# lauraset/Super-resolution-building-height-estimation

Measured on AMD Instinct MI355X. Metric: tiles/sec (64x64x8ch->256x256 height), higher is better.
Workload: dtype f16 operands / f32 accumulate (MFMA), f32 residual stream; 1 GPU; RRDBNet x4 (23 RRDB, 64 feat) forward_feature, batch 32 tiles/GPU, 64x64x3 -> 64x256x256 (BASELINE.json configs[1]); global_batch=32, parallelism=tile-sharded x1 (no data-path collective)

## Files before the change

### include/srbh.h

```cpp
#ifndef SRBH_H
#define SRBH_H

#include <stddef.h>
#include <stdint.h>

#ifdef __cplusplus
extern "C" {
#endif

#define SRBH_OK 0
#define SRBH_ERR_ARG (-1)
#define SRBH_ERR_WORKSPACE (-2)

int srbh_version(void);
const char* srbh_last_error(void);
#define SRBH_PATH_HCONV16 0
#define SRBH_PATH_HCONV_TEMPLATE 1
#define SRBH_PATH_ENTRY_FUSED 2
#define SRBH_PATH_ENTRY_SPLIT 3
#define SRBH_PATH_WGRAD16 4
#define SRBH_PATH_WGRAD_B16_GENERIC 5
#define SRBH_PATH_WGRAD_F32 6
#define SRBH_PATH_WGRAD_ENTRY_FUSED 7
#define SRBH_PATH_WGRAD_ENTRY_SPLIT 8
// ... 108 lines not shown
int srbh_rrdbnet_trunk_train_forward_persistent(const srbh_rrdbnet_desc* d, float* xr, float* xrr, void* dense_all, size_t dense_stride, int B, int H,
                                                int W, void* aux, void* stream, int* used);
size_t srbh_rrdbnet_trunk_wgrad_ws_bytes(void);
int srbh_rrdbnet_trunk_train_backward(int num_block, const void* dense_all, size_t dense_stride, const void* packs, size_t pack_stride,
                                      const size_t* pack_off, float* g_a, float* g_b, float* g_c, float** g_out, void* G, size_t g_stride,
                                      float* dw_all, float* db_all, float* wgrad_ws, int B, int H, int W, void* stream);
int srbh_rrdbnet_trunk_train_backward_persistent(int num_block, const void* dense_all, size_t dense_stride, const void* packs, size_t pack_stride,
                                                 const size_t* pack_off, const float* zero_bias, const float* g_a, float* g_b, float* g_c,
                                                 float** g_out, void* G_all, size_t g_stride, float* dw_all, float* db_all, float* wgrad_ws,
                                                 void* trunk_wgrad_ws, int B, int H, int W, void* aux, void* stream, int* used);
size_t srbh_trunk_wgrad_ws_bytes(int num_block, int B, int H, int W);
int srbh_trunk_wgrad(int num_block, const void* dense_all, size_t dense_stride, const void* G_all, size_t g_stride, int B, int H, int W, float* dw_all,
                     float* db_all, void* ws, void* stream);

int srbh_rrdbnet_last_status(const void* ws, int B, int H, int W, int want_forward, void* stream);

int srbh_rrdbnet_trunk_out(const void* ws, size_t ws_bytes, int num_block, int B, int H, int W, int want_forward, float* out, void* stream);

int srbh_ptail_wgs_cap(int cap);

int srbh_trunk_timing(int on);
int srbh_trunk_last_ms(float* ms);
const char* srbh_trunk_kernel_name(void);

size_t srbh_hpack_bytes(int cout, int cin, int ksize);
int srbh_hpack_conv_f32(const float* w_oihw, int cout, int cin, int ksize, int transpose_flip, float* packed, void* stream);

size_t srbh_bn_stats_bytes(int C);
int srbh_hconv_up_supported(int H, int W);

// ... 295 lines not shown
```

### super-resolution-building-height-estimation_amd/_lib.py

```python
from __future__ import annotations

import ctypes as C
import os
import subprocess
import threading

_HERE = os.path.dirname(os.path.abspath(__file__))
ROOT = os.path.dirname(_HERE)
CSRC = os.path.join(_HERE, "csrc")
INCLUDE = os.path.join(ROOT, "include")
LIB_PATH = os.path.join(_HERE, "libsrbh.so")
_DEV_LIB = os.environ.get("SRBH_LIB_PATH")
SOURCES = ["srbh_conv3x3.hip", "srbh_aux.hip", "srbh_rrdbnet.hip", "srbh_ptrunk.hip", "srbh_trunk_wgrad.hip", "srbh_ptail.hip", "srbh_ptail_split.hip", "srbh_head.hip", "srbh_head_bwd.hip", "srbh_mosaic.hip", "srbh_loader.hip", "srbh_loss.hip", "srbh_dwconv.hip", "srbh_mbconv.hip", "srbh_pwconv.hip", "srbh_dconv.hip", "srbh_optim.hip"]
HIPCC = os.environ.get("HIPCC", "/opt/rocm/bin/hipcc")
HIPFLAGS = ["--offload-arch=gfx950", "-O3", "-std=c++17", "-fPIC", "-Wno-unused-result", "-Wno-inline-asm"]
if os.environ.get("SRBH_HIPFLAGS_OVERRIDE"):
    HIPFLAGS = os.environ["SRBH_HIPFLAGS_OVERRIDE"].split()


def build(force: bool = False, verbose: bool = False) -> str:
    srcs = [os.path.join(CSRC, s) for s in SOURCES if os.path.exists(os.path.join(CSRC, s))]
    deps = srcs + [os.path.join(CSRC, f) for f in os.listdir(CSRC) if f.endswith(".h")] + [os.path.join(INCLUDE, "srbh.h")]
    if not force and os.path.exists(LIB_PATH) and all(os.path.getmtime(LIB_PATH) >= os.path.getmtime(d) for d in deps):
        return LIB_PATH
# ... 251 lines not shown
    "srbh_transpose_many": (_i, [_vp, _i, _vp]),
    "srbh_pwconv_bwd_data": (_i, [_vp, _vp, _vp, _i, _i, _i, _i, _vp]),
    "srbh_pwconv_bwd_data_res": (_i, [_vp, _vp, _vp, _vp, _i, _i, _i, _i, _vp]),
    "srbh_pwconv_bwd_weight_ws_floats": (_sz, [_i, _i, _i, _i]),
    "srbh_pwconv_bwd_weight": (_i, [_vp, _vp, _vp, _vp, _i, _i, _i, _i, _vp]),
    "srbh_dwconv_fwd": (_i, [_vp, _vp, _vp] + [_i] * 10 + [_vp]),
    "srbh_dwconv_bwd_data": (_i, [_vp, _vp, _vp] + [_i] * 10 + [_vp]),
    "srbh_dwconv_bwd_weight_splits": (_i, [_i, _i]),
    "srbh_dwconv_bwd_weight": (_i, [_vp, _vp, _vp, _vp] + [_i] * 10 + [_vp]),
    "srbh_mosaic_accumulate": (_i, [_vp, _vp, _i, _i, _i, _i, _vp, _vp, _vp, _vp, _i, _i, _vp]),
    "srbh_mosaic_finalize": (_i, [_vp, _vp, _vp, _i, _i, _i, _vp, _vp, _vp]),
    "srbh_label_prep": (_i, [_vp, _i, _i, _i, _vp, _vp, _vp, _vp, _vp, _vp, _vp, _vp]),
    "srbh_normalize_clamp": (_i, [_vp, _vp, _i, _i, _i, _i, _vp, _vp, _f, _f, _i, _vp]),
    "srbh_rrdbnet_workspace_bytes": (_sz, [_i, _i, _i, _i]),
    "srbh_rrdbnet_last_status": (_i, [_vp, _i, _i, _i, _i, _vp]),
    "srbh_rrdbnet_trunk_out": (_i, [_vp, _sz, _i, _i, _i, _i, _i, _vp, _vp]),
    "srbh_ptail_wgs_cap": (_i, [_i]),
    "srbh_wmse_sum": (_i, [_vp, _vp, _vp, C.c_long, _vp, _vp]),
    "srbh_wmse_grad": (_i, [_vp, _vp, _vp, C.c_long, _vp, _vp, _vp]),
    "srbh_cedice_sums": (_i, [_vp, _i, _i, C.c_long, C.c_long, C.c_long, C.c_long, _vp, _vp, _vp, _vp]),
    "srbh_cedice_grad": (_i, [_vp, _i, _i, C.c_long, C.c_long, C.c_long, C.c_long, _vp, _vp, _vp, _vp, _vp]),
    "srbh_height_metric_sums": (_i, [_vp, _vp, _vp, C.c_long, _i, _vp, _vp]),
    "srbh_confusion_add": (_i, [_vp, _vp, C.c_long, _i, _vp, _vp, _vp]),
    "srbh_trunk_timing": (_i, [_i]),
    "srbh_trunk_last_ms": (_i, [C.POINTER(C.c_float)]),
    "srbh_trunk_kernel_name": (C.c_char_p, []),
    "srbh_rrdbnet_forward": (_i, [C.POINTER(RRDBNetDesc), _vp, _vp, _i, _i, _i, _i, _vp, _sz, _vp]),
}

_lib = None
# ... 50 lines not shown
```

### super-resolution-building-height-estimation_amd/csrc/srbh_aux.hip

```cpp
#include "srbh_internal.h"

namespace srbh {

static thread_local char g_err[512] = "";

unsigned long long g_path_counters[PATH_N] = {};
void set_error(const char* fmt, ...) {
    va_list ap;
    va_start(ap, fmt);
    vsnprintf(g_err, sizeof(g_err), fmt, ap);
    va_end(ap);
}

int hip_fail(hipError_t e, const char* what) {
    set_error("HIP error %d (%s) in %s", (int)e, hipGetErrorString(e), what);
    return (int)e;
}

__global__ void zero_words_kernel(unsigned* __restrict__ p, size_t n) {
    size_t i = (size_t)blockIdx.x * blockDim.x + threadIdx.x;
    const size_t stride = (size_t)gridDim.x * blockDim.x;
    for (; i < n; i += stride) p[i] = 0u;
}

// ... 156 lines not shown
#pragma unroll
    for (int k = 0; k < 8; ++k) {
        float a = acc[k];
#pragma unroll
        for (int m = 4; m < 64; m <<= 1) a += __shfl_xor(a, m);
        if ((threadIdx.x & 63) < 4) atomicAdd(&red[oct * 8 + k], a);
    }
    __syncthreads();
    if (threadIdx.x < 32) atomicAdd(out + chunk * 32 + threadIdx.x, red[threadIdx.x]);
}

template <int CIN, int BF16 = 0>
__global__ __launch_bounds__(256) void conv_first_kernel(const float* __restrict__ x, const float* __restrict__ w,
                                                         const float* __restrict__ bias, int B, int cin_rt, int H, int W,
                                                         float* ra, float* rb, float* rc, char* out16, int row_b,
                                                         int plane_b, long img_b) {
    extern __shared__ float s_w[];
    const int cin = CIN > 0 ? CIN : cin_rt;
    for (int u = threadIdx.x; u < cin * 9 * 64; u += 256) {
        const int oc = u & 63, k = u >> 6;
        s_w[u] = w[(long)oc * cin * 9 + k];
    }
    __syncthreads();
    const int wq = (W + 3) >> 2;
    const long idx = (long)blockIdx.x * 256 + threadIdx.x;
    const long total = (long)B * H * wq * 16;
    if (idx >= total) return;
    const int og = idx & 15;
    long r = idx >> 4;
    const int xg = r % wq; r /= wq;
    const int yy = r % H;
    const int b = r / H;
// ... 278 lines not shown
    const int gx = (int)((npix + 255) / 256 < 1024 ? (npix + 255) / 256 : 1024);
    const char* base = (const char*)src + (long)chunk0 * g.plane_b;
    if (bf16) hipLaunchKernelGGL(act16_channel_sum_kernel<1>, dim3(gx, nchunk), dim3(256), 0, (hipStream_t)stream, base, B, H, W, nchunk, g.row_b, g.plane_b, g.img_b, out);
    else hipLaunchKernelGGL(act16_channel_sum_kernel<0>, dim3(gx, nchunk), dim3(256), 0, (hipStream_t)stream, base, B, H, W, nchunk, g.row_b, g.plane_b, g.img_b, out);
    SRBH_HIP(hipGetLastError());
    return SRBH_OK;
}

extern "C" int srbh_conv_first_f32(const float* x, const float* w, const float* bias, int B, int cin, int H, int W,
                                   float* ra, float* rb, float* rc, void* out16, int out16_chunks_total,
                                   void* stream) {
    return srbh::conv_first_f32(x, w, bias, B, cin, H, W, ra, rb, rc, out16, out16_chunks_total, 0, stream);
}

int srbh::conv_first_f32(const float* x, const float* w, const float* bias, int B, int cin, int H, int W, float* ra, float* rb, float* rc,
                         void* out16, int out16_chunks_total, int bf16, void* stream) {
    SRBH_REQUIRE(x && w && B > 0 && cin > 0 && H > 0 && W > 0, "srbh_conv_first_f32: bad arguments");
    SRBH_REQUIRE(!out16 || out16_chunks_total >= 2, "srbh_conv_first_f32: out16 needs >= 2 chunk planes");
    Act16Geo g = act16_geo(B, out16_chunks_total > 0 ? out16_chunks_total : 2, H, W);
    SRBH_REQUIRE(cin <= 56, "srbh_conv_first_f32: at most 56 input channels (got %d)", cin);
    long total = (long)B * H * ((W + 3) / 4) * 16;
    const size_t lds = (size_t)cin * 9 * 64 * sizeof(float);
    if (cin == 3 && bf16)
        hipLaunchKernelGGL((conv_first_kernel<3, 1>), dim3((total + 255) / 256), dim3(256), lds, (hipStream_t)stream, x, w, bias,
                           B, cin, H, W, ra, rb, rc, (char*)out16, g.row_b, g.plane_b, g.img_b);
    else if (cin == 3)
        hipLaunchKernelGGL(conv_first_kernel<3>, dim3((total + 255) / 256), dim3(256), lds, (hipStream_t)stream, x, w, bias,
                           B, cin, H, W, ra, rb, rc, (char*)out16, g.row_b, g.plane_b, g.img_b);
    else if (bf16) {
        if (lds > 65536)
            SRBH_ONCE_PER_DEVICE(SRBH_HIP(hipFuncSetAttribute((const void*)conv_first_kernel<0, 1>, hipFuncAttributeMaxDynamicSharedMemorySize, 56 * 9 * 64 * 4)));
        hipLaunchKernelGGL((conv_first_kernel<0, 1>), dim3((total + 255) / 256), dim3(256), lds, (hipStream_t)stream, x, w, bias,
                           B, cin, H, W, ra, rb, rc, (char*)out16, g.row_b, g.plane_b, g.img_b);
    } else {
        if (lds > 65536)
            SRBH_ONCE_PER_DEVICE(SRBH_HIP(hipFuncSetAttribute((const void*)conv_first_kernel<0>, hipFuncAttributeMaxDynamicSharedMemorySize, 56 * 9 * 64 * 4)));
        hipLaunchKernelGGL(conv_first_kernel<0>, dim3((total + 255) / 256), dim3(256), lds, (hipStream_t)stream, x, w, bias,
                           B, cin, H, W, ra, rb, rc, (char*)out16, g.row_b, g.plane_b, g.img_b);
    }
    SRBH_HIP(hipGetLastError());
    return SRBH_OK;
}
```

### super-resolution-building-height-estimation_amd/csrc/srbh_internal.h

```cpp
#pragma once
#include <hip/hip_runtime.h>
#include <stdarg.h>
#include <stdio.h>
#include <vector>
#include "srbh.h"

namespace srbh {

constexpr int PIX_B = 64;
constexpr int CHUNK_C = 32;
constexpr int TILE_W = 64;
constexpr int TILE_H = 8;

void set_error(const char* fmt, ...);
enum PathCounter { PATH_HCONV16 = 0, PATH_HCONV_TEMPLATE, PATH_ENTRY_FUSED, PATH_ENTRY_SPLIT, PATH_WGRAD16, PATH_WGRAD_B16_GENERIC,
                   PATH_WGRAD_F32, PATH_WGRAD_ENTRY_FUSED, PATH_WGRAD_ENTRY_SPLIT, PATH_HCONV_UP, PATH_HBWD16, PATH_HBLOCK16, PATH_N };
extern unsigned long long g_path_counters[PATH_N];
inline void count_path(int i) { ++g_path_counters[i]; }
int zero_async(void* p, size_t bytes, hipStream_t st);
int hip_fail(hipError_t e, const char* what);

#define SRBH_HIP(call)                                         \
    do {                                                       \
        hipError_t e_ = (call);                                \
// ... 27 lines not shown
};
inline Act16Geo act16_geo(int B, int chunks, int H, int W) {
    Act16Geo g;
    g.row_b = (W + 2) * PIX_B;
    g.plane_b = (H + 2) * g.row_b;
    g.img_b = (long)chunks * g.plane_b;
    size_t slack = (size_t)(TILE_H + 4) * (size_t)((W + 2 > TILE_W + 2) ? (W + 2) : (TILE_W + 2)) * PIX_B + 8192;
    g.total_b = (size_t)B * g.img_b + slack;
    g.total_b = (g.total_b + 255) & ~(size_t)255;
    return g;
}


size_t ptrunk_aux_bytes(int B, int tiles_per_img);
size_t ptrunk_err_offset(int B, int tiles_per_img);
int ptail_run(const srbh_conv3x3_args* a, hipStream_t stream, int* used);
int ptrunk_takes(int num_block, int H, int W, int* takes, int* ncu_out);
int ptrunk_run(const srbh_rrdbnet_desc* d, void* dense0, void* dense1, float* xr, float* xrr, int B, int H, int W,
               void* aux, hipStream_t stream, int* used, int* final_cur, long train_stride = 0, const void* mask = nullptr, long mask_stride = 0,
               bool bf16 = false);
int conv3x3_trunk_b16(const srbh_conv3x3_args* a, int out_f16, void* stream);
int conv_first_f32(const float* x, const float* w, const float* bias, int B, int cin, int H, int W, float* ra, float* rb, float* rc,
                   void* out16, int out16_chunks_total, int bf16, void* stream);


#if defined(__HIP_DEVICE_COMPILE__) || defined(__HIPCC__)
__device__ __forceinline__ void fold_stat_slots(double* stats, const int C, const int clear, double* red, double& s, double& q) {
    constexpr int NS = 64;
    const int t = threadIdx.x, V = 2 * C, G = 256 / V, v = t % V, g = t / V;
    double part = 0.0;
    if (g < G) {
        for (int k = g; k < NS; k += G) part += stats[(long)k * V + v];
        if (clear)
            for (int k = g; k < NS; k += G) stats[(long)k * V + v] = 0.0;
        red[g * V + v] = part;
    }
    __syncthreads();
    s = 0.0;
// ... 17 lines not shown
```

### super-resolution-building-height-estimation_amd/csrc/srbh_ptail.hip

```cpp
#include <stdlib.h>
#include "srbh_conv3x3_kernel.h"

namespace {
using namespace srbh;
using namespace srbh_k;

struct TParams {
    const char* in;
    long in_img_b;
    int in_plane_b, in_row_b;
    const char* w;
    const float* bias;
    int H, W;
    int tiles_x, tiles_per_img, ntiles, tiles_per_wg;
    int lrelu;
    char* out16;
    long out16_img_b;
    int out16_plane_b, out16_row_b;
    int out16_pix_b, out16_border;
    float* out32;
};

constexpr int W_RES_B = 2 * 36 * 1024;

template <int UPS>
__global__ __launch_bounds__(256, 1) void ptail_kernel(const TParams p) {
    using G = TileGeo<UPS>;
    constexpr int IN_EX = G::UNITS * 16;
    constexpr int CB = 2;
    extern __shared__ __attribute__((aligned(16))) char smem[];
    const int tid = threadIdx.x;
    const int lane = tid & 63;
    const int wave = __builtin_amdgcn_readfirstlane(tid >> 6);
    const int l31 = lane & 31, hi = lane >> 5;
    const int wr = wave >> 1, wc = wave & 1;
// ... 45 lines not shown
    };

    const int nst = ((p.H & (TILE_H - 1)) == 0 && (p.W & (TILE_W - 1)) == 0) ? (p.out32 ? 32 : 0) + (p.out16 ? 16 : 0) : 0;
    const int t0 = blockIdx.x * p.tiles_per_wg;
    const int t1 = (t0 + p.tiles_per_wg < p.ntiles) ? t0 + p.tiles_per_wg : p.ntiles;
    if (t0 >= t1) return;
#pragma unroll
    for (int k = 0; k < 18; ++k) dma16(p.w + (wave + 4 * k) * 1024 + lane * 16, (wave + 4 * k) * 1024, ~0ull);
    stage_inputs(t0);
    floatx4 bias4[CB][4];
#pragma unroll
    for (int mb = 0; mb < CB; ++mb)
#pragma unroll
        for (int g = 0; g < 4; ++g)
            bias4[mb][g] = p.bias ? *(const floatx4*)(p.bias + mb * 32 + g * 8 + hi * 4) : floatx4{0.f, 0.f, 0.f, 0.f};

    for (int t = t0; t < t1; ++t) {
        int img, Y0, X0;
        tile_origin(t, img, Y0, X0);
        if (t == t0 || nst == 0) asm volatile("s_waitcnt vmcnt(0)" ::: "memory");
        else if (nst == 16) asm volatile("s_waitcnt vmcnt(16)" ::: "memory");
        else if (nst == 32) asm volatile("s_waitcnt vmcnt(32)" ::: "memory");
        else asm volatile("s_waitcnt vmcnt(48)" ::: "memory");
        __syncthreads();
        floatx16 acc[CB][4];
#pragma unroll
        for (int mb = 0; mb < CB; ++mb)
#pragma unroll
            for (int i = 0; i < 4; ++i)
#pragma unroll
// ... 110 lines not shown
    hipLaunchKernelGGL(ptail_kernel<UPS>, dim3(grid), dim3(256), LDS_B, stream, p);
    SRBH_HIP(hipGetLastError());
    return SRBH_OK;
}

}

extern "C" int srbh_ptail_wgs_cap(int cap) {
    const int prev = g_ptail_wgs_cap;
    g_ptail_wgs_cap = cap > 0 ? cap : 0;
    return prev;
}

namespace srbh {

int ptail_run(const srbh_conv3x3_args* a, hipStream_t stream, int* used) {
    *used = 0;
    const char* e = getenv("SRBH_PTAIL");
    if (e && e[0] == '0') return SRBH_OK;
    if (a->in_chunks != 2 || a->cout != 64 || a->res1 || a->res2 || a->skip) return SRBH_OK;
    if (a->out32 && a->out32_c != 64) return SRBH_OK;
    const int tiles_x = (a->W + TILE_W - 1) / TILE_W, tiles_y = (a->H + TILE_H - 1) / TILE_H;
    if (a->out16_nhwc && (!a->out16 || a->out32)) return SRBH_OK;
    if ((long)tiles_x * tiles_y * a->B < 512 && !a->out16_nhwc) return SRBH_OK;
    const int inH = a->upsample2x ? a->H / 2 : a->H, inW = a->upsample2x ? a->W / 2 : a->W;
    const Act16Geo gi = act16_geo(a->B, a->in_chunks_total, inH, inW);
    TParams p{};
    p.in = (const char*)a->in + (long)a->in_chunk0 * gi.plane_b;
    p.in_img_b = gi.img_b;
    p.in_plane_b = gi.plane_b;
    p.in_row_b = gi.row_b;
// ... 11 lines not shown
        p.out16_pix_b = C * 2;
        p.out16_row_b = a->W * C * 2;
        p.out16_img_b = (long)a->H * a->W * C * 2;
        p.out16_plane_b = 64;
        p.out16_border = 0;
    } else if (a->out16) {
        const Act16Geo go = act16_geo(a->B, a->out16_chunks_total, a->H, a->W);
        p.out16_pix_b = PIX_B;
        p.out16_border = 1;
        p.out16 = (char*)a->out16 + (long)a->out16_chunk0 * go.plane_b;
        p.out16_img_b = go.img_b;
        p.out16_plane_b = go.plane_b;
        p.out16_row_b = go.row_b;
    }
    p.out32 = a->out32;
    const int rc = a->upsample2x ? launch<1>(p, stream) : launch<0>(p, stream);
    if (rc == SRBH_OK) *used = 1;
    return rc;
}

}
```

### super-resolution-building-height-estimation_amd/csrc/srbh_ptrunk.hip

```cpp
#include <stdlib.h>
#include <string.h>
#include <mutex>
#include "srbh_conv3x3_kernel.h"


namespace {
using namespace srbh;
using namespace srbh_k;

struct PLayer {
    const char* w;
    const float* bias;
};

struct PParams {
    char* dense[2];
    long img_b;
    int plane_b, row_b;
    float* xr;
    float* xrr;
    const PLayer* layers;
    int nlayers;
    int H, W, tiles_per_img, nblocks;
    int* prog;
    int* err;
    int* xcc;
    int force_wt;
    unsigned long long* prof;
    long dense_stride;
    int keep_all;
    int out_pixel;
    const char* mask;
    long mask_stride;
};

// ... 20 lines not shown
static int g_trunk_ev_recorded = 0;
static const char* g_trunk_kernel = "none";

constexpr int MAX_BLOCKS = 64;
static size_t table_bytes() { return ((size_t)MAX_BLOCKS * 15 * sizeof(PLayer) + 255) & ~(size_t)255; }
static size_t prog_bytes(int B, int tpi) { return ((size_t)B * 2 * tpi * sizeof(int) + 255) & ~(size_t)255; }

size_t ptrunk_aux_bytes(int B, int tiles_per_img) { return table_bytes() + 2 * prog_bytes(B, tiles_per_img) + 256; }
__global__ void ptrunk_reset_kernel(int* __restrict__ prog, int* __restrict__ xcc, int* __restrict__ err, int n) {
    const int i = blockIdx.x * blockDim.x + threadIdx.x;
    if (i < n) { prog[i] = 0; xcc[i] = 0; }
    if (i == 0) *err = 0;
}

size_t ptrunk_err_offset(int B, int tiles_per_img) { return table_bytes() + prog_bytes(B, tiles_per_img); }

struct TabEntry {
    int dev;
    std::vector<char> host;
    PLayer* dptr;
};
static std::mutex g_tab_mu;
static std::vector<TabEntry> g_tabs;

static int device_table(const std::vector<PLayer>& tab, PLayer** out) {
    int dev = 0;
    SRBH_HIP(hipGetDevice(&dev));
    const size_t nb = tab.size() * sizeof(PLayer);
    std::lock_guard<std::mutex> lock(g_tab_mu);
    for (size_t i = 0; i < g_tabs.size(); ++i)
// ... 27 lines not shown
    constexpr int LDS_B = P_LDS_B;
    SRBH_ONCE_PER_DEVICE({
        SRBH_HIP(hipFuncSetAttribute((const void*)ptrunk3_kernel<0>, hipFuncAttributeMaxDynamicSharedMemorySize, LDS_B));
        SRBH_HIP(hipFuncSetAttribute((const void*)ptrunk3_kernel<1>, hipFuncAttributeMaxDynamicSharedMemorySize, LDS_B));
        SRBH_HIP(hipFuncSetAttribute((const void*)ptrunk3_kernel<0, 1>, hipFuncAttributeMaxDynamicSharedMemorySize, LDS_B));
        SRBH_HIP(hipFuncSetAttribute((const void*)ptrunk3_kernel<0, 0, 1>, hipFuncAttributeMaxDynamicSharedMemorySize, LDS_B));
    });
    int per_cu = 0;
    SRBH_HIP(hipOccupancyMaxActiveBlocksPerMultiprocessor(&per_cu, ptrunk3_kernel<0>, 256, LDS_B));
    if (per_cu < 1) return SRBH_OK;
    *takes = 1;
    return SRBH_OK;
}

int ptrunk_run(const srbh_rrdbnet_desc* d, void* dense0, void* dense1, float* xr, float* xrr, int B, int H, int W,
               void* aux, hipStream_t stream, int* used, int* final_cur, long train_stride, const void* mask, long mask_stride, bool bf16) {
    *used = 0;
    if (mask && train_stride <= 0) return SRBH_OK;
    SRBH_REQUIRE(!bf16 || (train_stride == 0 && !mask), "ptrunk_run: the bf16 form is the inference forward only");
    int ncu = 0, takes = 0;
    if (int rc = ptrunk_takes(d->num_block, H, W, &takes, &ncu)) return rc;
    if (!takes) return SRBH_OK;
    const int tpi = H / TILE_H;
    constexpr int LDS_B = P_LDS_B;
    const int nl = d->num_block * 15;
    std::vector<PLayer> tab(nl);
    int cur = 0, li = 0;
    for (int blk = 0; blk < d->num_block; ++blk)
        for (int r = 0; r < 3; ++r) {
            const srbh_conv_w* cw = d->rdb + (blk * 3 + r) * 5;
            for (int k = 0; k < 5; ++k) tab[li++] = PLayer{(const char*)cw[k].w, cw[k].bias};
            cur ^= 1;
        }
    *final_cur = cur;
    char* a = (char*)aux;
    PLayer* d_tab = nullptr;
    if (int rc = device_table(tab, &d_tab)) return rc;
    int* d_prog = (int*)(a + table_bytes());
    int* d_err = (int*)(a + ptrunk_err_offset(B, tpi));
    int* d_xcc = (int*)(a + ptrunk_err_offset(B, tpi) + 256);
    hipLaunchKernelGGL(ptrunk_reset_kernel, dim3((B * tpi + 255) / 256), dim3(256), 0, stream, d_prog, d_xcc, d_err, B * tpi);
    SRBH_HIP(hipGetLastError());
    const Act16Geo g = act16_geo(B, 6, H, W);
    int imgs_per_launch = ncu / tpi;
    if (const char* ie = getenv("SRBH_PT_IMAGES")) {
        const int cap = atoi(ie);
        if (cap > 0 && cap < imgs_per_launch) {
            const int nl_ = (B + cap - 1) / cap;
            imgs_per_launch = (B + nl_ - 1) / nl_;
        }
    }
    for (int b0 = 0; b0 < B; b0 += imgs_per_launch) {
        const int nb = (B - b0) < imgs_per_launch ? (B - b0) : imgs_per_launch;
        PParams pp;
        pp.dense_stride = train_stride;
        pp.keep_all = pp.out_pixel = train_stride > 0;
        pp.mask = mask ? (const char*)mask + (long)b0 * g.img_b : nullptr;
        pp.mask_stride = mask_stride;
        pp.dense[0] = (char*)dense0 + (long)b0 * g.img_b;
        pp.dense[1] = (train_stride > 0 ? (char*)dense0 + train_stride : (char*)dense1) + (long)b0 * g.img_b;
        pp.img_b = g.img_b;
        pp.plane_b = g.plane_b;
        pp.row_b = g.row_b;
        pp.xr = xr + (long)b0 * H * W * 64;
        pp.xrr = xrr + (long)b0 * H * W * 64;
        pp.layers = d_tab;
        pp.nlayers = nl;
        pp.H = H;
        pp.W = W;
        pp.tiles_per_img = tpi;
        pp.nblocks = nb * tpi;
        pp.prog = d_prog + b0 * tpi;
        pp.err = d_err;
        pp.xcc = d_xcc + b0 * tpi;
        {
            const char* e = getenv("SRBH_PT_WT");
            pp.force_wt = (e && atoi(e) == 1) ? 1 : 0;
        }
        if (getenv("SRBH_PT_PROF") && !bf16 && !g_ptrunk_prof)
            SRBH_HIP(hipMalloc(&g_ptrunk_prof, (size_t)ncu * MAX_BLOCKS * 15 * 6 * 8));
// ... 79 lines not shown
```

### super-resolution-building-height-estimation_amd/csrc/srbh_ptrunk3_kernel.h

```cpp
#pragma once

#ifndef P3_S1
#define P3_S1 1
#endif
#ifndef P3_X2REG
#define P3_X2REG 1
#endif
#ifndef P3_SKIPST
#define P3_SKIPST 1
#endif
#ifndef P3_LAZYDRAIN
#define P3_LAZYDRAIN 1
#endif

#ifndef P3_SEAM
#define P3_SEAM 1
#endif


#ifndef P3_PREREAD
#define P3_PREREAD 1
#endif
#ifndef P3_TRAIN
#define P3_TRAIN 1
// ... 155 lines not shown
            if (wt)
                __hip_atomic_store(pp.prog + t, v, __ATOMIC_RELAXED, __HIP_MEMORY_SCOPE_AGENT);
            else
                __hip_atomic_store(pp.prog + t, v, __ATOMIC_RELAXED, __HIP_MEMORY_SCOPE_WORKGROUP);
        }
    };
    bool pending_pub = false;
    int pub_val = 0;

    floatx4 xres[2][4][4];
    const int X = wc * 32 + l31;
    {
#pragma unroll
        for (int i = 0; i < 4; ++i) {
            const int Y = Y0 + wr * 4 + i;
            const float* q = pp.xrr + (((long)img * pp.H + Y) * pp.W + X) * 64 + hi * 4;
#pragma unroll
            for (int mb = 0; mb < 2; ++mb)
#pragma unroll
                for (int g = 0; g < 4; ++g) xres[mb][i][g] = *(const floatx4*)(q + mb * 32 + g * 8);
        }
    }

    typedef unsigned uintx4 __attribute__((ext_vector_type(4)));
    uintx4 x1p[4][2], X1r[4][2], X2r[4][2];
    const int soff = (wr * 4 + 1) * G::ROW_B + (X + 1) * PIX_B;
    const int sswz[2] = {((0 + hi) ^ (((X + 1) >> 2) & 3)) << 4, ((2 + hi) ^ (((X + 1) >> 2) & 3)) << 4};
    const int boff = (wr * 5 + (lane >> 2)) * G::ROW_B + (wc ? (G::COLS - 1) * PIX_B : 0) + (lane & 3) * 16;
    int hoff[2];
    {
        const int px = 1 + (tid >> 2), ps = tid & 3;
// ... 314 lines not shown
                    asm volatile("global_store_dwordx4 %0, %1, off\n\ts_nop 1" ::"v"(o), "v"(raw) : "memory");
            }
        }
    };
    auto epi64 = [&](floatx16 (&acc)[2][4], char* obase, const bool r2, const bool r2_pixel, const bool x1_halo_only, const bool keep, const bool out_px,
                     const bool f16out) {
        floatx4 bias4[2][4];
#pragma unroll
        for (int mb = 0; mb < 2; ++mb)
#pragma unroll
            for (int g = 0; g < 4; ++g) bias4[mb][g] = *(const floatx4*)((const float*)(smem + B_BIAS_OFF) + mb * 32 + g * 8 + hi * 4);
        const int frag_lane = wc * 2048 + lane * 4;
        floatx4 a2[2][2][4];
        auto load_a2 = [&](const int slot, const int i) {
            const long rowb = ((long)img * pp.H + Y0 + wr * 4 + i) * pp.W * 64;
            const float* q2 = pp.xrr + rowb + (r2_pixel ? X * 64 + hi * 4 : frag_lane);
            const int sm = r2_pixel ? 32 : 1024, sg = r2_pixel ? 8 : 256;
#pragma unroll
            for (int mb = 0; mb < 2; ++mb)
#pragma unroll
                for (int g = 0; g < 4; ++g) a2[slot][mb][g] = *(const floatx4*)(q2 + mb * sm + g * sg);
        };
#pragma unroll
        for (int io = 0; io < 4; ++io) {
            const int i = io == 0 ? 0 : io == 1 ? 3 : io - 1;
            if (r2 && io == 1) load_a2(0, 0);
            if (r2 && io == 2) load_a2(1, 3);
            const bool halo = (i == 0 && wr == 0) || (i == 3 && wr == 1);
#pragma unroll
            for (int mb = 0; mb < 2; ++mb) {
#pragma unroll
// ... 213 lines not shown
```

### super-resolution-building-height-estimation_amd/csrc/srbh_rrdbnet.hip

```cpp
#include <stdlib.h>
#include "srbh_internal.h"

using namespace srbh;

namespace {

struct WsLayout {
    size_t d0, d1, feat, xr, xrr, u2, u3, u4, aux, total;
    size_t u2lo, u3lo;
    size_t dense_b;
};

inline size_t align256(size_t v) { return (v + 255) & ~(size_t)255; }

__global__ __launch_bounds__(256) void poison_on_error_kernel(const int* __restrict__ err, float* __restrict__ out, size_t n) {
    if (__hip_atomic_load(err, __ATOMIC_RELAXED, __HIP_MEMORY_SCOPE_AGENT) == 0) return;
    const float nan = __builtin_nanf("");
    for (size_t i = (size_t)blockIdx.x * blockDim.x + threadIdx.x; i < n; i += (size_t)gridDim.x * blockDim.x) out[i] = nan;
}

__global__ __launch_bounds__(256) void trunk_out_pixel_order_kernel(const float* __restrict__ src, float* __restrict__ dst, long nquads) {
    typedef float f4 __attribute__((ext_vector_type(4)));
    for (long i = (long)blockIdx.x * blockDim.x + threadIdx.x; i < nquads; i += (long)gridDim.x * blockDim.x) {
        const long row = i >> 10;
        const int f = (int)(i & 1023);
        const int lane = f & 63, g = (f >> 6) & 3, mb = (f >> 8) & 1, wc = f >> 9;
        const int px = wc * 32 + (lane & 31);
        ((f4*)dst)[row * 1024 + px * 16 + mb * 8 + g * 2 + (lane >> 5)] = ((const f4*)src)[i];
    }
}

inline bool persistent_wanted() {
    const char* env = getenv("SRBH_PERSISTENT");
    return !(env && env[0] == '0');
}

WsLayout ws_layout(int B, int H, int W, int want_forward, bool f16x2 = false) {
    WsLayout L;
    size_t off = 0;
    L.dense_b = act16_geo(B, 6, H, W).total_b;
    L.d0 = off; off = align256(off + L.dense_b);
    L.d1 = off; off = align256(off + L.dense_b);
    size_t res_b = (size_t)B * H * W * 64 * sizeof(float);
    L.feat = off; off = align256(off + res_b);
    L.xr = off; off = align256(off + res_b);
// ... 41 lines not shown
    }
    char* base = (char*)ws;
    void* D[2] = {base + L.d0, base + L.d1};
    float* feat = (float*)(base + L.feat);
    float* xr = (float*)(base + L.xr);
    float* xrr = (float*)(base + L.xrr);
    void* U2 = base + L.u2;
    void* U3 = base + L.u3;
    void* U4 = base + L.u4;

    bool bf16 = false;
    if (d->rdb_b16 && d->num_block > 0) {
        const char* env = getenv("SRBH_TRUNK_BF16");
        bf16 = !(env && env[0] == '0');
    }
    int rc = conv_first_f32(x, d->conv_first_w, d->conv_first_b, B, d->num_in_ch, H, W, feat, xr, xrr, D[0], 6, bf16 ? 1 : 0, stream);
    if (rc) return rc;

    srbh_conv3x3_args a;
    int cur = 0;
    int used_persistent = 0;
    {
        if (persistent_wanted()) {
            srbh_rrdbnet_desc dt = *d;
            if (bf16) dt.rdb = d->rdb_b16;
            rc = ptrunk_run(&dt, D[0], D[1], xr, xrr, B, H, W, base + L.aux, (hipStream_t)stream, &used_persistent, &cur, 0, nullptr, 0, bf16);
            if (rc) return rc;
        }
    }
    for (int blk = 0; !used_persistent && blk < d->num_block; ++blk) {
        for (int r = 0; r < 3; ++r) {
            const srbh_conv_w* cw = (bf16 ? d->rdb_b16 : d->rdb) + (blk * 3 + r) * 5;
            for (int k = 0; k < 4; ++k) {
                a = srbh_conv3x3_args{};
                a.in = D[cur]; a.in_chunks_total = 6; a.in_chunk0 = 0; a.in_chunks = 2 + k;
                a.w = cw[k].w; a.bias = cw[k].bias; a.cout = 32;
                a.B = B; a.H = H; a.W = W; a.lrelu = 1;
                a.out16 = D[cur]; a.out16_chunks_total = 6; a.out16_chunk0 = 2 + k;
                if ((rc = bf16 ? conv3x3_trunk_b16(&a, 0, stream) : srbh_conv3x3_f16(&a, stream))) return rc;
            }
            a = srbh_conv3x3_args{};
            a.in = D[cur]; a.in_chunks_total = 6; a.in_chunk0 = 0; a.in_chunks = 6;
            a.w = cw[4].w; a.bias = cw[4].bias; a.cout = 64;
            a.B = B; a.H = H; a.W = W;
            a.res_scale = 0.2f; a.res1 = xr; a.res1_update = 1;
            if (r == 2) { a.res2 = xrr; a.res2_scale = 0.2f; a.res2_update = 1; }
            a.out16 = D[cur ^ 1]; a.out16_chunks_total = 6; a.out16_chunk0 = 0;
            const bool last = blk + 1 == d->num_block && r == 2;
            if ((rc = bf16 ? conv3x3_trunk_b16(&a, last ? 1 : 0, stream) : srbh_conv3x3_f16(&a, stream))) return rc;
            cur ^= 1;
        }
    }
    const int* err_word = (const int*)(base + L.aux + ptrunk_err_offset(B, (H + TILE_H - 1) / TILE_H));
    auto guard = [&](int out_c) -> int {
        if (!used_persistent) return SRBH_OK;
        hipLaunchKernelGGL(poison_on_error_kernel, dim3(1024), dim3(256), 0, (hipStream_t)stream, err_word, out,
                           (size_t)B * 16 * H * W * out_c);
        SRBH_HIP(hipGetLastError());
        return SRBH_OK;
    };
    if (split) {
        if ((rc = srbh_act16_split_lo(xrr, used_persistent, D[cur], 6, 0, D[cur], 6, 2, B, H, W, stream))) return rc;
        srbh_conv3x3_split s;
        a = srbh_conv3x3_args{};
        s = srbh_conv3x3_split{};
        a.in = D[cur]; a.in_chunks_total = 6; a.in_chunk0 = 0; a.in_chunks = 2;
        s.in_lo = D[cur]; s.in_lo_chunks_total = 6; s.in_lo_chunk0 = 2;
        a.w = d->conv_body.w; s.w_lo = d->conv_body_lo; a.bias = d->conv_body.bias; a.cout = 64;
        a.B = B; a.H = H; a.W = W; a.skip = feat;
        a.out16 = D[cur ^ 1]; a.out16_chunks_total = 6; a.out16_chunk0 = 0;
        s.out16_lo = D[cur ^ 1]; s.out16_lo_chunks_total = 6; s.out16_lo_chunk0 = 2;
        if ((rc = srbh_conv3x3_f16x2(&a, &s, stream))) return rc;
        a = srbh_conv3x3_args{};
        s = srbh_conv3x3_split{};
        a.in = D[cur ^ 1]; a.in_chunks_total = 6; a.in_chunk0 = 0; a.in_chunks = 2;
        s.in_lo = D[cur ^ 1]; s.in_lo_chunks_total = 6; s.in_lo_chunk0 = 2;
        a.w = d->conv_up1.w; s.w_lo = d->conv_up1_lo; a.bias = d->conv_up1.bias; a.cout = 64;
// ... 31 lines not shown
    a.in = D[cur ^ 1]; a.in_chunks_total = 6; a.in_chunk0 = 0; a.in_chunks = 2;
    a.w = d->conv_up1.w; a.bias = d->conv_up1.bias; a.cout = 64;
    a.B = B; a.H = 2 * H; a.W = 2 * W; a.upsample2x = 1; a.lrelu = 1;
    a.out16 = U2; a.out16_chunks_total = 2; a.out16_chunk0 = 0;
    if ((rc = srbh_conv3x3_f16(&a, stream))) return rc;
    a = srbh_conv3x3_args{};
    a.in = U2; a.in_chunks_total = 2; a.in_chunk0 = 0; a.in_chunks = 2;
    a.w = d->conv_up2.w; a.bias = d->conv_up2.bias; a.cout = 64;
    a.B = B; a.H = 4 * H; a.W = 4 * W; a.upsample2x = 1; a.lrelu = 1;
    a.out16 = U3; a.out16_chunks_total = 2; a.out16_chunk0 = 0;
    if ((rc = srbh_conv3x3_f16(&a, stream))) return rc;
    a = srbh_conv3x3_args{};
    a.in = U3; a.in_chunks_total = 2; a.in_chunk0 = 0; a.in_chunks = 2;
    a.w = d->conv_hr.w; a.bias = d->conv_hr.bias; a.cout = 64;
    a.B = B; a.H = 4 * H; a.W = 4 * W;
    if (want_forward == 2) {
        a.out16 = out; a.out16_chunks_total = 2; a.out16_chunk0 = 0; a.out16_nhwc = 1;
        if ((rc = srbh_conv3x3_f16(&a, stream))) return rc;
        return guard(32);
    }
    if (!want_forward) {
        a.out32 = out; a.out32_c = 64;
        if ((rc = srbh_conv3x3_f16(&a, stream))) return rc;
        return guard(64);
    }
    a.lrelu = 1;
    a.out16 = U4; a.out16_chunks_total = 2; a.out16_chunk0 = 0;
    if ((rc = srbh_conv3x3_f16(&a, stream))) return rc;
    SRBH_REQUIRE(d->conv_last.w && d->num_out_ch >= 1 && d->num_out_ch <= 32,
                 "srbh_rrdbnet_forward: conv_last needs 1..32 output channels (got %d)", d->num_out_ch);
    a = srbh_conv3x3_args{};
    a.in = U4; a.in_chunks_total = 2; a.in_chunk0 = 0; a.in_chunks = 2;
    a.w = d->conv_last.w; a.bias = d->conv_last.bias; a.cout = 32;
    a.B = B; a.H = 4 * H; a.W = 4 * W;
    a.out32 = out; a.out32_c = d->num_out_ch;
    if ((rc = srbh_conv3x3_f16(&a, stream))) return rc;
    return guard(d->num_out_ch);
}

extern "C" int srbh_rrdbnet_trunk_out(const void* ws, size_t ws_bytes, int num_block, int B, int H, int W, int want_forward, float* out,
                                      void* stream) {
    SRBH_REQUIRE(ws && out && B > 0 && H > 0 && W > 0 && num_block >= 0, "srbh_rrdbnet_trunk_out: bad arguments");
    const WsLayout L = ws_layout(B, H, W, want_forward);
    if (ws_bytes < L.total) {
        set_error("srbh_rrdbnet_trunk_out: workspace %zu bytes < required %zu", ws_bytes, L.total);
        return SRBH_ERR_WORKSPACE;
    }
    const float* xrr = (const float*)((const char*)ws + L.xrr);
    const size_t n = (size_t)B * H * W * 64;
    int fragment = 0;
    if (persistent_wanted()) {
        if (int rc = ptrunk_takes(num_block, H, W, &fragment, nullptr)) return rc;
    }
    if (!fragment) {
        SRBH_HIP(hipMemcpyAsync(out, xrr, n * sizeof(float), hipMemcpyDeviceToDevice, (hipStream_t)stream));
        return SRBH_OK;
    }
    const long nquads = (long)(n / 4);
    hipLaunchKernelGGL(trunk_out_pixel_order_kernel, dim3((unsigned)((nquads + 255) / 256)), dim3(256), 0, (hipStream_t)stream, xrr, out, nquads);
    SRBH_HIP(hipGetLastError());
    return SRBH_OK;
}

extern "C" int srbh_rrdbnet_last_status(const void* ws, int B, int H, int W, int want_forward, void* stream) {
    SRBH_REQUIRE(ws && B > 0 && H > 0 && W > 0, "srbh_rrdbnet_last_status: bad arguments");
    const WsLayout L = ws_layout(B, H, W, want_forward);
    const int tpi = (H + TILE_H - 1) / TILE_H;
    SRBH_HIP(hipStreamSynchronize((hipStream_t)stream));
    int err = 0;
    const size_t eoff = ptrunk_err_offset(B, tpi);
    SRBH_HIP(hipMemcpy(&err, (const char*)ws + L.aux + eoff, sizeof(int), hipMemcpyDeviceToHost));
    if (err) set_error("persistent trunk kernel timed out waiting for a neighbour workgroup (err=%d)", err);
    return err ? -3 : SRBH_OK;
}

// ... 232 lines not shown
```

Baseline: 8046 tiles/s.

## Fold trunk reset into conv_first, skip residual copies, fuse tail error guard

Clears the persistent-trunk progress, xcc and error words inside conv_first_kernel, which removes the separate reset launch. When the persistent trunk runs, conv_first stops writing the xr/xrr f32 copies and the trunk reads the original features through a new x0 pointer. The final conv now goes through ptail_run, which reads the error word and writes NaN bias on error, so the separate poison kernel is skipped when the tail path is taken. It also adds a test hook that can pin the error word, and this adds coupling between stages.

```diff
diff --git a/include/srbh.h b/include/srbh.h
--- a/include/srbh.h
+++ b/include/srbh.h
@@ -146,6 +146,8 @@
                      float* db_all, void* ws, void* stream);
 
 int srbh_rrdbnet_last_status(const void* ws, int B, int H, int W, int want_forward, void* stream);
+
+int srbh_rrdbnet_hold_error_word(void* ws, int B, int H, int W, int want_forward, int value, int hold, void* stream);
 
 int srbh_rrdbnet_trunk_out(const void* ws, size_t ws_bytes, int num_block, int B, int H, int W, int want_forward, float* out, void* stream);
 
diff --git a/super-resolution-building-height-estimation_amd/_lib.py b/super-resolution-building-height-estimation_amd/_lib.py
--- a/super-resolution-building-height-estimation_amd/_lib.py
+++ b/super-resolution-building-height-estimation_amd/_lib.py
@@ -289,6 +289,7 @@
     "srbh_normalize_clamp": (_i, [_vp, _vp, _i, _i, _i, _i, _vp, _vp, _f, _f, _i, _vp]),
     "srbh_rrdbnet_workspace_bytes": (_sz, [_i, _i, _i, _i]),
     "srbh_rrdbnet_last_status": (_i, [_vp, _i, _i, _i, _i, _vp]),
+    "srbh_rrdbnet_hold_error_word": (_i, [_vp, _i, _i, _i, _i, _i, _i, _vp]),
     "srbh_rrdbnet_trunk_out": (_i, [_vp, _sz, _i, _i, _i, _i, _i, _vp, _vp]),
     "srbh_ptail_wgs_cap": (_i, [_i]),
     "srbh_wmse_sum": (_i, [_vp, _vp, _vp, C.c_long, _vp, _vp]),
diff --git a/super-resolution-building-height-estimation_amd/csrc/srbh_aux.hip b/super-resolution-building-height-estimation_amd/csrc/srbh_aux.hip
--- a/super-resolution-building-height-estimation_amd/csrc/srbh_aux.hip
+++ b/super-resolution-building-height-estimation_amd/csrc/srbh_aux.hip
@@ -194,8 +194,15 @@
 __global__ __launch_bounds__(256) void conv_first_kernel(const float* __restrict__ x, const float* __restrict__ w,
                                                          const float* __restrict__ bias, int B, int cin_rt, int H, int W,
                                                          float* ra, float* rb, float* rc, char* out16, int row_b,
-                                                         int plane_b, long img_b) {
+                                                         int plane_b, long img_b, const srbh::PtrunkClear clr) {
     extern __shared__ float s_w[];
+    if (clr.n > 0) {
+        for (long i = (long)blockIdx.x * 256 + threadIdx.x; i < clr.n; i += (long)gridDim.x * 256) {
+            clr.prog[i] = 0;
+            clr.xcc[i] = 0;
+        }
+        if (clr.err && blockIdx.x == 0 && threadIdx.x == 0) *clr.err = 0;
+    }
     const int cin = CIN > 0 ? CIN : cin_rt;
     for (int u = threadIdx.x; u < cin * 9 * 64; u += 256) {
         const int oc = u & 63, k = u >> 6;
@@ -504,7 +511,8 @@
 }
 
 int srbh::conv_first_f32(const float* x, const float* w, const float* bias, int B, int cin, int H, int W, float* ra, float* rb, float* rc,
-                         void* out16, int out16_chunks_total, int bf16, void* stream) {
+                         void* out16, int out16_chunks_total, int bf16, void* stream, const PtrunkClear* clr_in) {
+    const PtrunkClear clr = clr_in ? *clr_in : PtrunkClear{};
     SRBH_REQUIRE(x && w && B > 0 && cin > 0 && H > 0 && W > 0, "srbh_conv_first_f32: bad arguments");
     SRBH_REQUIRE(!out16 || out16_chunks_total >= 2, "srbh_conv_first_f32: out16 needs >= 2 chunk planes");
     Act16Geo g = act16_geo(B, out16_chunks_total > 0 ? out16_chunks_total : 2, H, W);
@@ -513,21 +521,21 @@
     const size_t lds = (size_t)cin * 9 * 64 * sizeof(float);
     if (cin == 3 && bf16)
         hipLaunchKernelGGL((conv_first_kernel<3, 1>), dim3((total + 255) / 256), dim3(256), lds, (hipStream_t)stream, x, w, bias,
-                           B, cin, H, W, ra, rb, rc, (char*)out16, g.row_b, g.plane_b, g.img_b);
+                           B, cin, H, W, ra, rb, rc, (char*)out16, g.row_b, g.plane_b, g.img_b, clr);
     else if (cin == 3)
         hipLaunchKernelGGL(conv_first_kernel<3>, dim3((total + 255) / 256), dim3(256), lds, (hipStream_t)stream, x, w, bias,
-                           B, cin, H, W, ra, rb, rc, (char*)out16, g.row_b, g.plane_b, g.img_b);
+                           B, cin, H, W, ra, rb, rc, (char*)out16, g.row_b, g.plane_b, g.img_b, clr);
     else if (bf16) {
         if (lds > 65536)
             SRBH_ONCE_PER_DEVICE(SRBH_HIP(hipFuncSetAttribute((const void*)conv_first_kernel<0, 1>, hipFuncAttributeMaxDynamicSharedMemorySize, 56 * 9 * 64 * 4)));
         hipLaunchKernelGGL((conv_first_kernel<0, 1>), dim3((total + 255) / 256), dim3(256), lds, (hipStream_t)stream, x, w, bias,
-                           B, cin, H, W, ra, rb, rc, (char*)out16, g.row_b, g.plane_b, g.img_b);
+                           B, cin, H, W, ra, rb, rc, (char*)out16, g.row_b, g.plane_b, g.img_b, clr);
     } else {
         if (lds > 65536)
             SRBH_ONCE_PER_DEVICE(SRBH_HIP(hipFuncSetAttribute((const void*)conv_first_kernel<0>, hipFuncAttributeMaxDynamicSharedMemorySize, 56 * 9 * 64 * 4)));
         hipLaunchKernelGGL(conv_first_kernel<0>, dim3((total + 255) / 256), dim3(256), lds, (hipStream_t)stream, x, w, bias,
-                           B, cin, H, W, ra, rb, rc, (char*)out16, g.row_b, g.plane_b, g.img_b);
-    }
-    SRBH_HIP(hipGetLastError());
-    return SRBH_OK;
-}
+                           B, cin, H, W, ra, rb, rc, (char*)out16, g.row_b, g.plane_b, g.img_b, clr);
+    }
+    SRBH_HIP(hipGetLastError());
+    return SRBH_OK;
+}
diff --git a/super-resolution-building-height-estimation_amd/csrc/srbh_internal.h b/super-resolution-building-height-estimation_amd/csrc/srbh_internal.h
--- a/super-resolution-building-height-estimation_amd/csrc/srbh_internal.h
+++ b/super-resolution-building-height-estimation_amd/csrc/srbh_internal.h
@@ -65,14 +65,21 @@
 
 size_t ptrunk_aux_bytes(int B, int tiles_per_img);
 size_t ptrunk_err_offset(int B, int tiles_per_img);
-int ptail_run(const srbh_conv3x3_args* a, hipStream_t stream, int* used);
+struct PtrunkClear {
+    int* prog = nullptr;
+    int* xcc = nullptr;
+    int* err = nullptr;
+    int n = 0;
+};
+PtrunkClear ptrunk_clear_words(void* aux, int B, int tiles_per_img);
+int ptail_run(const srbh_conv3x3_args* a, hipStream_t stream, int* used, const int* err = nullptr);
 int ptrunk_takes(int num_block, int H, int W, int* takes, int* ncu_out);
 int ptrunk_run(const srbh_rrdbnet_desc* d, void* dense0, void* dense1, float* xr, float* xrr, int B, int H, int W,
                void* aux, hipStream_t stream, int* used, int* final_cur, long train_stride = 0, const void* mask = nullptr, long mask_stride = 0,
-               bool bf16 = false);
+               bool bf16 = false, const float* x0 = nullptr, bool cleared = false);
 int conv3x3_trunk_b16(const srbh_conv3x3_args* a, int out_f16, void* stream);
 int conv_first_f32(const float* x, const float* w, const float* bias, int B, int cin, int H, int W, float* ra, float* rb, float* rc,
-                   void* out16, int out16_chunks_total, int bf16, void* stream);
+                   void* out16, int out16_chunks_total, int bf16, void* stream, const PtrunkClear* clr = nullptr);
 
 
 #if defined(__HIP_DEVICE_COMPILE__) || defined(__HIPCC__)
diff --git a/super-resolution-building-height-estimation_amd/csrc/srbh_ptail.hip b/super-resolution-building-height-estimation_amd/csrc/srbh_ptail.hip
--- a/super-resolution-building-height-estimation_amd/csrc/srbh_ptail.hip
+++ b/super-resolution-building-height-estimation_amd/csrc/srbh_ptail.hip
@@ -19,6 +19,7 @@
     int out16_plane_b, out16_row_b;
     int out16_pix_b, out16_border;
     float* out32;
+    const int* err;
 };
 
 constexpr int W_RES_B = 2 * 36 * 1024;
@@ -94,6 +95,13 @@
 #pragma unroll
         for (int g = 0; g < 4; ++g)
             bias4[mb][g] = p.bias ? *(const floatx4*)(p.bias + mb * 32 + g * 8 + hi * 4) : floatx4{0.f, 0.f, 0.f, 0.f};
+    if (p.err && __hip_atomic_load(p.err, __ATOMIC_RELAXED, __HIP_MEMORY_SCOPE_AGENT) != 0) {
+        const float nan = __builtin_nanf("");
+#pragma unroll
+        for (int mb = 0; mb < CB; ++mb)
+#pragma unroll
+            for (int g = 0; g < 4; ++g) bias4[mb][g] = floatx4{nan, nan, nan, nan};
+    }
 
     for (int t = t0; t < t1; ++t) {
         int img, Y0, X0;
@@ -234,7 +242,7 @@
 
 namespace srbh {
 
-int ptail_run(const srbh_conv3x3_args* a, hipStream_t stream, int* used) {
+int ptail_run(const srbh_conv3x3_args* a, hipStream_t stream, int* used, const int* err) {
     *used = 0;
     const char* e = getenv("SRBH_PTAIL");
     if (e && e[0] == '0') return SRBH_OK;
@@ -276,6 +284,7 @@
         p.out16_row_b = go.row_b;
     }
     p.out32 = a->out32;
+    p.err = err;
     const int rc = a->upsample2x ? launch<1>(p, stream) : launch<0>(p, stream);
     if (rc == SRBH_OK) *used = 1;
     return rc;
diff --git a/super-resolution-building-height-estimation_amd/csrc/srbh_ptrunk.hip b/super-resolution-building-height-estimation_amd/csrc/srbh_ptrunk.hip
--- a/super-resolution-building-height-estimation_amd/csrc/srbh_ptrunk.hip
+++ b/super-resolution-building-height-estimation_amd/csrc/srbh_ptrunk.hip
@@ -19,6 +19,7 @@
     int plane_b, row_b;
     float* xr;
     float* xrr;
+    const float* x0;
     const PLayer* layers;
     int nlayers;
     int H, W, tiles_per_img, nblocks;
@@ -69,6 +70,16 @@
 }
 
 size_t ptrunk_err_offset(int B, int tiles_per_img) { return table_bytes() + prog_bytes(B, tiles_per_img); }
+
+PtrunkClear ptrunk_clear_words(void* aux, int B, int tiles_per_img) {
+    char* a = (char*)aux;
+    PtrunkClear c;
+    c.prog = (int*)(a + table_bytes());
+    c.err = (int*)(a + ptrunk_err_offset(B, tiles_per_img));
+    c.xcc = (int*)(a + ptrunk_err_offset(B, tiles_per_img) + 256);
+    c.n = B * tiles_per_img;
+    return c;
+}
 
 struct TabEntry {
     int dev;
@@ -126,7 +137,8 @@
 }
 
 int ptrunk_run(const srbh_rrdbnet_desc* d, void* dense0, void* dense1, float* xr, float* xrr, int B, int H, int W,
-               void* aux, hipStream_t stream, int* used, int* final_cur, long train_stride, const void* mask, long mask_stride, bool bf16) {
+               void* aux, hipStream_t stream, int* used, int* final_cur, long train_stride, const void* mask, long mask_stride, bool bf16,
+               const float* x0, bool cleared) {
     *used = 0;
     if (mask && train_stride <= 0) return SRBH_OK;
     SRBH_REQUIRE(!bf16 || (train_stride == 0 && !mask), "ptrunk_run: the bf16 form is the inference forward only");
@@ -148,11 +160,14 @@
     char* a = (char*)aux;
     PLayer* d_tab = nullptr;
     if (int rc = device_table(tab, &d_tab)) return rc;
-    int* d_prog = (int*)(a + table_bytes());
-    int* d_err = (int*)(a + ptrunk_err_offset(B, tpi));
-    int* d_xcc = (int*)(a + ptrunk_err_offset(B, tpi) + 256);
-    hipLaunchKernelGGL(ptrunk_reset_kernel, dim3((B * tpi + 255) / 256), dim3(256), 0, stream, d_prog, d_xcc, d_err, B * tpi);
-    SRBH_HIP(hipGetLastError());
+    const PtrunkClear cw = ptrunk_clear_words(a, B, tpi);
+    int* d_prog = cw.prog;
+    int* d_err = cw.err;
+    int* d_xcc = cw.xcc;
+    if (!cleared) {
+        hipLaunchKernelGGL(ptrunk_reset_kernel, dim3((B * tpi + 255) / 256), dim3(256), 0, stream, d_prog, d_xcc, d_err, B * tpi);
+        SRBH_HIP(hipGetLastError());
+    }
     const Act16Geo g = act16_geo(B, 6, H, W);
     int imgs_per_launch = ncu / tpi;
     if (const char* ie = getenv("SRBH_PT_IMAGES")) {
@@ -176,6 +191,7 @@
         pp.row_b = g.row_b;
         pp.xr = xr + (long)b0 * H * W * 64;
         pp.xrr = xrr + (long)b0 * H * W * 64;
+        pp.x0 = (x0 ? x0 : xrr) + (long)b0 * H * W * 64;
         pp.layers = d_tab;
         pp.nlayers = nl;
         pp.H = H;
diff --git a/super-resolution-building-height-estimation_amd/csrc/srbh_ptrunk3_kernel.h b/super-resolution-building-height-estimation_amd/csrc/srbh_ptrunk3_kernel.h
--- a/super-resolution-building-height-estimation_amd/csrc/srbh_ptrunk3_kernel.h
+++ b/super-resolution-building-height-estimation_amd/csrc/srbh_ptrunk3_kernel.h
@@ -193,7 +193,7 @@
 #pragma unroll
         for (int i = 0; i < 4; ++i) {
             const int Y = Y0 + wr * 4 + i;
-            const float* q = pp.xrr + (((long)img * pp.H + Y) * pp.W + X) * 64 + hi * 4;
+            const float* q = pp.x0 + (((long)img * pp.H + Y) * pp.W + X) * 64 + hi * 4;
 #pragma unroll
             for (int mb = 0; mb < 2; ++mb)
 #pragma unroll
@@ -538,7 +538,7 @@
         floatx4 a2[2][2][4];
         auto load_a2 = [&](const int slot, const int i) {
             const long rowb = ((long)img * pp.H + Y0 + wr * 4 + i) * pp.W * 64;
-            const float* q2 = pp.xrr + rowb + (r2_pixel ? X * 64 + hi * 4 : frag_lane);
+            const float* q2 = (r2_pixel ? pp.x0 : (const float*)pp.xrr) + rowb + (r2_pixel ? X * 64 + hi * 4 : frag_lane);
             const int sm = r2_pixel ? 32 : 1024, sg = r2_pixel ? 8 : 256;
 #pragma unroll
             for (int mb = 0; mb < 2; ++mb)
diff --git a/super-resolution-building-height-estimation_amd/csrc/srbh_rrdbnet.hip b/super-resolution-building-height-estimation_amd/csrc/srbh_rrdbnet.hip
--- a/super-resolution-building-height-estimation_amd/csrc/srbh_rrdbnet.hip
+++ b/super-resolution-building-height-estimation_amd/csrc/srbh_rrdbnet.hip
@@ -29,6 +29,8 @@
         ((f4*)dst)[row * 1024 + px * 16 + mb * 8 + g * 2 + (lane >> 5)] = ((const f4*)src)[i];
     }
 }
+
+int g_hold_error_word = 0;
 
 inline bool persistent_wanted() {
     const char* env = getenv("SRBH_PERSISTENT");
@@ -100,8 +102,18 @@
         const char* env = getenv("SRBH_TRUNK_BF16");
         bf16 = !(env && env[0] == '0');
     }
-    int rc = conv_first_f32(x, d->conv_first_w, d->conv_first_b, B, d->num_in_ch, H, W, feat, xr, xrr, D[0], 6, bf16 ? 1 : 0, stream);
+    int will_persist = 0;
+    if (persistent_wanted()) {
+        if (int rc0 = ptrunk_takes(d->num_block, H, W, &will_persist, nullptr)) return rc0;
+    }
+    const int tpi = (H + TILE_H - 1) / TILE_H;
+    PtrunkClear clr = ptrunk_clear_words(base + L.aux, B, tpi);
+    if (g_hold_error_word) clr.err = nullptr;
+    const bool per_layer = !will_persist && d->num_block > 0;
+    int rc = conv_first_f32(x, d->conv_first_w, d->conv_first_b, B, d->num_in_ch, H, W, feat, per_layer ? xr : nullptr, per_layer ? xrr : nullptr,
+                            D[0], 6, bf16 ? 1 : 0, stream, will_persist ? &clr : nullptr);
     if (rc) return rc;
+    const float* trunk32 = d->num_block > 0 ? xrr : feat;
 
     srbh_conv3x3_args a;
     int cur = 0;
@@ -110,8 +122,10 @@
         if (persistent_wanted()) {
             srbh_rrdbnet_desc dt = *d;
             if (bf16) dt.rdb = d->rdb_b16;
-            rc = ptrunk_run(&dt, D[0], D[1], xr, xrr, B, H, W, base + L.aux, (hipStream_t)stream, &used_persistent, &cur, 0, nullptr, 0, bf16);
+            rc = ptrunk_run(&dt, D[0], D[1], xr, xrr, B, H, W, base + L.aux, (hipStream_t)stream, &used_persistent, &cur, 0, nullptr, 0, bf16, feat,
+                            will_persist != 0);
             if (rc) return rc;
+            SRBH_REQUIRE(used_persistent == will_persist, "srbh_rrdbnet_forward: the persistent trunk changed its mind between two calls");
         }
     }
     for (int blk = 0; !used_persistent && blk < d->num_block; ++blk) {
@@ -137,7 +151,7 @@
             cur ^= 1;
         }
     }
-    const int* err_word = (const int*)(base + L.aux + ptrunk_err_offset(B, (H + TILE_H - 1) / TILE_H));
+    const int* err_word = (const int*)(base + L.aux + ptrunk_err_offset(B, tpi));
     auto guard = [&](int out_c) -> int {
         if (!used_persistent) return SRBH_OK;
         hipLaunchKernelGGL(poison_on_error_kernel, dim3(1024), dim3(256), 0, (hipStream_t)stream, err_word, out,
@@ -146,7 +160,7 @@
         return SRBH_OK;
     };
     if (split) {
-        if ((rc = srbh_act16_split_lo(xrr, used_persistent, D[cur], 6, 0, D[cur], 6, 2, B, H, W, stream))) return rc;
+        if ((rc = srbh_act16_split_lo(trunk32, used_persistent, D[cur], 6, 0, D[cur], 6, 2, B, H, W, stream))) return rc;
         srbh_conv3x3_split s;
         a = srbh_conv3x3_args{};
         s = srbh_conv3x3_split{};
@@ -208,15 +222,22 @@
     a.in = U3; a.in_chunks_total = 2; a.in_chunk0 = 0; a.in_chunks = 2;
     a.w = d->conv_hr.w; a.bias = d->conv_hr.bias; a.cout = 64;
     a.B = B; a.H = 4 * H; a.W = 4 * W;
+    auto last_conv = [&](int out_words) -> int {
+        int tail = 0;
+        if (used_persistent) {
+            if (int rc1 = ptail_run(&a, (hipStream_t)stream, &tail, err_word)) return rc1;
+        }
+        if (tail) return SRBH_OK;
+        if (int rc1 = srbh_conv3x3_f16(&a, stream)) return rc1;
+        return guard(out_words);
+    };
     if (want_forward == 2) {
         a.out16 = out; a.out16_chunks_total = 2; a.out16_chunk0 = 0; a.out16_nhwc = 1;
-        if ((rc = srbh_conv3x3_f16(&a, stream))) return rc;
-        return guard(32);
+        return last_conv(32);
     }
     if (!want_forward) {
         a.out32 = out; a.out32_c = 64;
-        if ((rc = srbh_conv3x3_f16(&a, stream))) return rc;
-        return guard(64);
+        return last_conv(64);
     }
     a.lrelu = 1;
     a.out16 = U4; a.out16_chunks_total = 2; a.out16_chunk0 = 0;
@@ -240,7 +261,7 @@
         set_error("srbh_rrdbnet_trunk_out: workspace %zu bytes < required %zu", ws_bytes, L.total);
         return SRBH_ERR_WORKSPACE;
     }
-    const float* xrr = (const float*)((const char*)ws + L.xrr);
+    const float* xrr = (const float*)((const char*)ws + (num_block > 0 ? L.xrr : L.feat));
     const size_t n = (size_t)B * H * W * 64;
     int fragment = 0;
     if (persistent_wanted()) {
@@ -253,6 +274,15 @@
     const long nquads = (long)(n / 4);
     hipLaunchKernelGGL(trunk_out_pixel_order_kernel, dim3((unsigned)((nquads + 255) / 256)), dim3(256), 0, (hipStream_t)stream, xrr, out, nquads);
     SRBH_HIP(hipGetLastError());
+    return SRBH_OK;
+}
+
+extern "C" int srbh_rrdbnet_hold_error_word(void* ws, int B, int H, int W, int want_forward, int value, int hold, void* stream) {
+    SRBH_REQUIRE(ws && B > 0 && H > 0 && W > 0, "srbh_rrdbnet_hold_error_word: bad arguments");
+    const WsLayout L = ws_layout(B, H, W, want_forward);
+    SRBH_HIP(hipStreamSynchronize((hipStream_t)stream));
+    SRBH_HIP(hipMemcpy((char*)ws + L.aux + ptrunk_err_offset(B, (H + TILE_H - 1) / TILE_H), &value, sizeof(int), hipMemcpyHostToDevice));
+    g_hold_error_word = hold ? 1 : 0;
     return SRBH_OK;
 }
 
```

Result: no change. 8089 tiles/s (median of 6 runs) (+0.5%).
